# JialeTao/MRFA

Measured on AMD Instinct MI355X. Metric: frames/sec (256x256 source+driving pair) fwd+bwd, higher is better.
Workload: dtype f32; 1 GPU; vox1.yaml MTIA (TokenPose_B) prior + DenseMotion + RaftFlow refinement, 256x256, bs=8/GPU, fwd+bwd+clip+Adam, train-mode BN, surrogate L1 loss; global_batch=8, parallelism=dp1, prior=mtia, background_predictor=False, sync_bn=False, launch=hipGraph, optimizer=FlatAdam (K20), mfma=bf16x6

## Files before the change

### mrfa_amd/csrc/wgrad_lean.hip

```cpp
#include <stdlib.h>
#include <type_traits>
#include "mfma_bf16.h"

namespace {

constexpr int WL_MAXP = 24;

struct LeanW {
    const float* x; const float* dy; float* dw;
    const float* in_scale; const float* in_shift;
    int ldx, ldy, N, H, W, Cin, Cout, groups;
    float alpha;
    int G;
    int Q;
};
struct LeanWMulti {
    int n;
    int prefix[WL_MAXP + 1];
    LeanW p[WL_MAXP];
};

template <int NB, int TW, bool PRO, int NP>
__global__ __launch_bounds__(256, 1) void wgrad_lean_kernel(const LeanWMulti a) {
    constexpr int NPXW = NB == 1 ? 4 : 1;
    constexpr int TR = 32 / TW, PR = NPXW * TR, HP = TW + 2, HPIX = (PR + 2) * HP, DPIX = NPXW * 32;
    constexpr int XBLK = HPIX * 64, DBLK = DPIX * 64;
    constexpr int NPC = NP == 6 ? 3 : (NP == 3 ? 2 : 1);
    constexpr int XPLANE = NB * XBLK, DPLANE = NB * DBLK;
    constexpr int NXU = NB * HPIX * 8, NDU = NB * DPIX * 8;
    constexpr int NX = (NXU + 255) / 256, ND = (NDU + 255) / 256;
    extern __shared__ __attribute__((aligned(16))) unsigned char smem[];
    constexpr int IMG = NPC * (XPLANE + DPLANE);

    const int tid = threadIdx.x, lane = tid & 63, wave = __builtin_amdgcn_readfirstlane(tid >> 6);
    int pi = 0;
    while (pi + 1 < a.n && (int)blockIdx.x >= a.prefix[pi + 1]) ++pi;
    const LeanW& p = a.p[pi];
    const int local = (int)blockIdx.x - a.prefix[pi];
    const int nci = p.Cin / (32 * NB);
    const int bg = local / p.G, jr = local - bg * p.G;
    const int co0 = (bg / nci) * (32 * NB), ci0 = (bg % nci) * (32 * NB);
    const int q0 = (int)((long long)jr * p.Q / p.G), q1 = (int)((long long)(jr + 1) * p.Q / p.G);
    const int tiles_x = p.W / TW, tiles_y = (p.H + PR - 1) / PR;
    const int wpx = NB == 1 ? wave : 0, wco = NB == 1 ? 0 : (wave >> 1), wci = NB == 1 ? 0 : (wave & 1);

    auto x_unit = [&](int j, int& blk, int& hp, int& quad) -> bool {
        const int u = tid + j * 256;
        const int uu = u < NXU ? u : 0;
        blk = uu / (HPIX * 8);
        const int rem = uu - blk * (HPIX * 8);
        hp = rem >> 3;
        quad = rem & 7;
        return u < NXU;
    };
    auto d_unit = [&](int j, int& blk, int& px, int& quad) -> bool {
        const int u = tid + j * 256;
        const int uu = u < NDU ? u : 0;
        blk = uu / (DPIX * 8);
        const int rem = uu - blk * (DPIX * 8);
        px = rem >> 3;
        quad = rem & 7;
        return u < NDU;
    };
    float* const smP = reinterpret_cast<float*>(smem + 2 * IMG);
    if constexpr (PRO) {
        const int G = p.groups > 1 ? p.groups : 1;
        for (int i = tid; i < G * 2 * 32 * NB; i += 256) {
            const int g = i / (2 * 32 * NB), r = i - g * (2 * 32 * NB), which = r / (32 * NB), c = r - which * (32 * NB);
            smP[i] = (which ? p.in_shift : p.in_scale)[g * p.Cin + ci0 + c];
        }
        __syncthreads();
    }

    f32x4 rx[NX], rd[ND];
    unsigned okmask = 0;
    int cur_grp = 0;
    auto load_patch = [&](int q) {
        const int tx = q % tiles_x;
        int t = q / tiles_x;
        const int ty = t % tiles_y, n = t / tiles_y;
        const int y0 = ty * PR, x0 = tx * TW;
        const float* xb = p.x + (size_t)n * p.H * p.W * p.ldx;
        const float* db = p.dy + (size_t)n * p.H * p.W * p.ldy;
        okmask = 0;
#pragma unroll
        for (int j = 0; j < NX; ++j) {
            int blk, hp, quad;
            const bool val = x_unit(j, blk, hp, quad);
            const int hy = hp / HP, hx = hp - hy * HP;
            const int iy = y0 - 1 + hy, ix = x0 - 1 + hx;
            const bool ok = val && (unsigned)iy < (unsigned)p.H && (unsigned)ix < (unsigned)p.W;
            okmask |= ok ? (1u << j) : 0u;
            rx[j] = *reinterpret_cast<const f32x4*>(xb + (size_t)(ok ? iy * p.W + ix : 0) * p.ldx + ci0 + blk * 32 + quad * 4);
        }
#pragma unroll
        for (int j = 0; j < ND; ++j) {
            int blk, px, quad;
            const bool val = d_unit(j, blk, px, quad);
            const int r = px / TW, c = px - r * TW;
            const int oy = y0 + r;
            const bool ok = val && oy < p.H;
            okmask |= ok ? (1u << (16 + j)) : 0u;
            rd[j] = *reinterpret_cast<const f32x4*>(db + (size_t)(ok ? oy * p.W + x0 + c : 0) * p.ldy + co0 + blk * 32 + quad * 4);
        }
        cur_grp = p.groups > 1 ? n / (p.N / p.groups) : 0;
    };
    auto store_unit = [&](int k, int buf) {
        const f32x4 z = {0.f, 0.f, 0.f, 0.f};
        unsigned char* const smX = smem + buf * IMG;
        unsigned char* const smD = smX + NPC * XPLANE;
        if (k < NX) {
            const int j = k;
            int blk, hp, quad;
            const bool val = x_unit(j, blk, hp, quad);
            f32x4 v = rx[j];
            if constexpr (PRO) {
                const float* ps = smP + cur_grp * (2 * 32 * NB) + blk * 32 + quad * 4;
                const f32x4 psc = *reinterpret_cast<const f32x4*>(ps), psh = *reinterpret_cast<const f32x4*>(ps + 32 * NB);
                v = v * psc + psh;
#pragma unroll
                for (int e = 0; e < 4; ++e) v[e] = fmaxf(v[e], 0.f);
            }
            v = (okmask >> j) & 1u ? v : z;
            u32x2 p1, p2, p3;
            bf16_pieces<NP>(v, p1, p2, p3);
            if (val) {
                unsigned char* dst = smX + blk * XBLK + hp * 64 + quad * 8;
                *reinterpret_cast<u32x2*>(dst) = p1;
                if constexpr (NPC >= 2) *reinterpret_cast<u32x2*>(dst + XPLANE) = p2;
                if constexpr (NPC == 3) *reinterpret_cast<u32x2*>(dst + 2 * XPLANE) = p3;
            }
        } else {
            const int j = k - NX;
            int blk, px, quad;
            const bool val = d_unit(j, blk, px, quad);
            const f32x4 v = (okmask >> (16 + j)) & 1u ? rd[j] : z;
            u32x2 p1, p2, p3;
            bf16_pieces<NP>(v, p1, p2, p3);
            if (val) {
                unsigned char* dst = smD + blk * DBLK + px * 64 + quad * 8;
                *reinterpret_cast<u32x2*>(dst) = p1;
                if constexpr (NPC >= 2) *reinterpret_cast<u32x2*>(dst + DPLANE) = p2;
                if constexpr (NPC == 3) *reinterpret_cast<u32x2*>(dst + 2 * DPLANE) = p3;
            }
        }
    };

    f32x16 acc[9];
#pragma unroll
    for (int t = 0; t < 9; ++t)
#pragma unroll
        for (int r = 0; r < 16; ++r) acc[t][r] = 0.f;

    const int l16 = lane & 15, grp16 = lane >> 4;
    const int frag_off = (8 * (grp16 >> 1) + (l16 >> 2)) * 64 + (grp16 & 1) * 32 + (l16 & 3) * 8;
    const int a_off = wco * DBLK + wpx * (32 * 64) + frag_off;
    const int b_off = wci * XBLK + frag_off;
    constexpr int TG = 3, NGRP = 3;
    constexpr int NUNIT = NX + ND, UPG = (NUNIT + 2 * NGRP - 1) / (2 * NGRP);
    auto compute = [&](int buf, bool stage) {
        const unsigned char* const smX = smem + buf * IMG;
        const unsigned char* const smD = smX + NPC * XPLANE;
#pragma unroll
        for (int kk = 0; kk < 2; ++kk) {
            const int row0 = TW == 32 ? wpx : wpx * 2 + kk, col0 = TW == 32 ? 16 * kk : 0;
            bf16x8 af[NPC];
#pragma unroll
            for (int pc = 0; pc < NPC; ++pc) af[pc] = tr_frag(smD + pc * DPLANE + a_off + kk * 16 * 64);
#pragma unroll
            for (int gi = 0; gi < NGRP; ++gi) {
                const int g0 = gi * TG;
                bf16x8 bfr[NPC][TG];
#pragma unroll
                for (int q = 0; q < TG; ++q) {
                    const int tap = g0 + q, r = tap / 3, s = tap - 3 * r;
#pragma unroll
                    for (int pc = 0; pc < NPC; ++pc) bfr[pc][q] = tr_frag(smX + pc * XPLANE + b_off + ((row0 + r) * HP + col0 + s) * 64);
                }
#pragma unroll
                for (int t = 6 - NP; t < 6; ++t)
#pragma unroll
                    for (int q = 0; q < TG; ++q) acc[g0 + q] = __builtin_amdgcn_mfma_f32_32x32x16_bf16(af[PA[t]], bfr[PB[t]][q], acc[g0 + q], 0, 0, 0);
                if (stage) {
#pragma unroll
                    for (int k = (kk * NGRP + gi) * UPG; k < (kk * NGRP + gi + 1) * UPG; ++k)
                        if (k < NUNIT) store_unit(k, buf ^ 1);
                }
            }
        }
    };

    if (q0 < q1) {
        load_patch(q0);
#pragma unroll
        for (int k = 0; k < NUNIT; ++k) store_unit(k, q0 & 1);
        if (q0 + 1 < q1) load_patch(q0 + 1);
        __syncthreads();
        for (int q = q0; q < q1; ++q) {
            const bool more = q + 1 < q1;
            compute(q & 1, more);
            if (q + 2 < q1) load_patch(q + 2);
            __syncthreads();
        }
    }

    if constexpr (NB == 1) {
        float* red = reinterpret_cast<float*>(smem);
        for (int w = 1; w < 4; ++w) {
            __syncthreads();
            if (wave == w) {
#pragma unroll
                for (int t = 0; t < 9; ++t)
#pragma unroll
                    for (int r = 0; r < 16; ++r) red[(t * 16 + r) * 64 + lane] = acc[t][r];
            }
            __syncthreads();
            if (wave == 0) {
#pragma unroll
                for (int t = 0; t < 9; ++t)
#pragma unroll
                    for (int r = 0; r < 16; ++r) acc[t][r] += red[(t * 16 + r) * 64 + lane];
            }
        }
        if (wave != 0) return;
    }
    if (q0 >= q1) return;
    const int ci = ci0 + wci * 32 + (lane & 31), half = lane >> 5;
#pragma unroll
    for (int t = 0; t < 9; ++t)
#pragma unroll
        for (int g = 0; g < 4; ++g)
#pragma unroll
            for (int e = 0; e < 4; ++e) {
                const int co = co0 + wco * 32 + 8 * g + 4 * half + e;
                atomicAdd(p.dw + ((size_t)t * p.Cout + co) * p.Cin + ci, p.alpha * acc[t][4 * g + e]);
            }
}

template <int NB, int TW>
constexpr size_t wl_lds(int npc) {
    constexpr int NPXW = NB == 1 ? 4 : 1, TR = 32 / TW, PR = NPXW * TR, HP = TW + 2, HPIX = (PR + 2) * HP, DPIX = NPXW * 32;
    const size_t st = (size_t)2 * npc * NB * (HPIX + DPIX) * 64 + (size_t)3 * 2 * 32 * NB * 4, red = NB == 1 ? (size_t)9 * 16 * 64 * 4 : 0;
    return st > red ? st : red;
}

int wl_variant(const mrfa_wgrad_params& p) {
    if (p.Cin == 32 && p.Cout == 32) return (p.Wout % 32) == 0 ? 0 : -1;
    if ((p.Cin % 64) || (p.Cout % 64)) return -1;
    return (p.Wout % 32) == 0 ? 1 : ((p.Wout % 16) == 0 ? 2 : -1);
}

template <int NB, int TW>
int wl_launch(hipStream_t st, const LeanWMulti& m, bool pro, int mode) {
    dim3 grid((unsigned)m.prefix[m.n]);
#define WL(PRO_, NP_)                                                                                                                              \
    do {                                                                                                                                          \
        constexpr size_t lds = wl_lds<NB, TW>(NP_ == 6 ? 3 : (NP_ == 3 ? 2 : 1));                                                                  \
        if constexpr (lds > 65536) {                                        \
            static const hipError_t attr = hipFuncSetAttribute(reinterpret_cast<const void*>(&wgrad_lean_kernel<NB, TW, PRO_, NP_>),               \
                                                               hipFuncAttributeMaxDynamicSharedMemorySize, (int)lds);                             \
            if (attr != hipSuccess) { mrfa_set_error("wgrad(lean): %zu bytes of LDS refused: %s", lds, hipGetErrorString(attr)); return 2; }      \
        }                                                                                                                                         \
        hipLaunchKernelGGL((wgrad_lean_kernel<NB, TW, PRO_, NP_>), grid, dim3(256), lds, st, m);                                                  \
    } while (0)
    if (mode == 3) { if (pro) WL(true, 1); else WL(false, 1); }
    else if (mode == 2) { if (pro) WL(true, 3); else WL(false, 3); }
    else { if (pro) WL(true, 6); else WL(false, 6); }
#undef WL
    return 0;
}

}

bool mrfa_wgrad_lean_eligible(const mrfa_wgrad_params& p) {
    const int mode = mrfa_get_mfma_mode();
    if (!g_tune.wgrad_lean || (mode != 1 && mode != 2 && mode != 3)) return false;
    if (p.kflat > 0 || p.ups || p.R != 3 || p.S != 3 || p.pad != 1 || p.nbatch > 1 || p.ksplit > 0 || p.stride > 1 || p.dbias) return false;
    if (p.Hout != p.Hin || p.Wout != p.Win || p.Cin > 128 || p.Cout > 128) return false;
    if ((p.ldx % 4) != 0 || !aligned16(p.x) || (p.ldy % 4) != 0 || !aligned16(p.dy)) return false;
    if (p.in_scale && (!p.in_relu || !aligned16(p.in_scale) || !aligned16(p.in_shift))) return false;
    if (p.groups > 1 && ((p.N % p.groups) != 0 || p.groups > 3)) return false;
    if ((long long)p.N * p.Hin * p.Win * p.ldx >= (1ll << 31) || (long long)p.N * p.Hout * p.Wout * p.ldy >= (1ll << 31)) return false;
    if (2.0 * (double)p.N * p.Hout * p.Wout * p.Cout * 9.0 * p.Cin > 2.6e9) return false;
    return wl_variant(p) >= 0;
}

int mrfa_wgrad_lean_multi(hipStream_t st, const mrfa_wgrad_params* ps, int n, unsigned char* taken) {
    const int mode = mrfa_get_mfma_mode();
    int neligible = 0;
    for (int i = 0; i < n; ++i) neligible += (taken[i] = mrfa_wgrad_lean_eligible(ps[i]) ? 1 : 0);
    if (!neligible) return 0;
    for (int v = 0; v < 3; ++v)
        for (int pro = 0; pro < 2; ++pro) {
            int idx[4096], cnt = 0;
            for (int i = 0; i < n && cnt < 4096; ++i)
                if (taken[i] && wl_variant(ps[i]) == v && (ps[i].in_scale != nullptr) == (pro != 0)) idx[cnt++] = i;
            for (int b0 = 0; b0 < cnt; b0 += WL_MAXP) {
                const int nb = cnt - b0 < WL_MAXP ? cnt - b0 : WL_MAXP;
                LeanWMulti m;
                m.n = nb;
                m.prefix[0] = 0;
                long long blocks = 0;
                for (int k = 0; k < nb; ++k) {
                    const mrfa_wgrad_params& q = ps[idx[b0 + k]];
                    blocks += v == 0 ? 1 : (q.Cin / 64) * (q.Cout / 64);
                }
                int G = (int)((512 + blocks - 1) / blocks);
                if (G > 64) G = 64;
                for (int k = 0; k < nb; ++k) {
                    const mrfa_wgrad_params& q = ps[idx[b0 + k]];
                    LeanW& w = m.p[k];
                    const int PR = v == 0 ? 4 : (v == 1 ? 1 : 2), TW = v == 2 ? 16 : 32;
                    w.x = q.x; w.dy = q.dy; w.dw = q.dw; w.in_scale = q.in_scale; w.in_shift = q.in_shift;
                    w.ldx = q.ldx; w.ldy = q.ldy; w.N = q.N; w.H = q.Hout; w.W = q.Wout; w.Cin = q.Cin; w.Cout = q.Cout; w.groups = q.groups;
                    w.alpha = q.alpha;
                    w.Q = q.N * (q.Wout / TW) * cdiv(q.Hout, PR);
                    w.G = G < w.Q ? G : w.Q;
                    const int nblocks = v == 0 ? 1 : (q.Cin / 64) * (q.Cout / 64);
                    m.prefix[k + 1] = m.prefix[k] + w.G * nblocks;
                }
                int rc = 0;
                if (v == 0) rc = wl_launch<1, 32>(st, m, pro != 0, mode);
                else if (v == 1) rc = wl_launch<2, 32>(st, m, pro != 0, mode);
                else rc = wl_launch<2, 16>(st, m, pro != 0, mode);
                if (rc) return rc;
                MRFA_CHECK_LAUNCH("mrfa_conv2d_wgrad_multi(lean)");
            }
        }
    return 0;
}
```

Before: 103.1 pairs/s.

## Split wgrad taps across two wave groups in 512-thread lean kernel

Doubles the lean weight-gradient workgroup to 512 threads. The 9 filter taps are split between two groups of four waves, one taking 5 taps and the other 4, which cuts per-wave accumulator registers from 9 to 5 tiles. For the NB=2 variants the pixel patch per iteration is doubled (two k-tiles), and the grid target is lowered to 256 workgroups so each block covers more patches. This aims to lift register pressure and improve latency hiding, at the cost of duplicated A-fragment loads across the tap groups, larger LDS tiles and fewer blocks in flight.

```diff
diff --git a/mrfa_amd/csrc/wgrad_lean.hip b/mrfa_amd/csrc/wgrad_lean.hip
--- a/mrfa_amd/csrc/wgrad_lean.hip
+++ b/mrfa_amd/csrc/wgrad_lean.hip
@@ -20,15 +20,20 @@
     LeanW p[WL_MAXP];
 };
 
+constexpr int WL_TARGET_WGS = 256;
+constexpr int WL_THREADS = 512;
+constexpr int WL_TAPS = 5;
+
 template <int NB, int TW, bool PRO, int NP>
-__global__ __launch_bounds__(256, 1) void wgrad_lean_kernel(const LeanWMulti a) {
+__global__ __launch_bounds__(WL_THREADS, 1) void wgrad_lean_kernel(const LeanWMulti a) {
     constexpr int NPXW = NB == 1 ? 4 : 1;
-    constexpr int TR = 32 / TW, PR = NPXW * TR, HP = TW + 2, HPIX = (PR + 2) * HP, DPIX = NPXW * 32;
+    constexpr int NKT = NB == 1 ? 1 : 2;
+    constexpr int TR = 32 / TW, PR = NPXW * NKT * TR, HP = TW + 2, HPIX = (PR + 2) * HP, DPIX = NPXW * NKT * 32;
     constexpr int XBLK = HPIX * 64, DBLK = DPIX * 64;
     constexpr int NPC = NP == 6 ? 3 : (NP == 3 ? 2 : 1);
     constexpr int XPLANE = NB * XBLK, DPLANE = NB * DBLK;
     constexpr int NXU = NB * HPIX * 8, NDU = NB * DPIX * 8;
-    constexpr int NX = (NXU + 255) / 256, ND = (NDU + 255) / 256;
+    constexpr int NX = (NXU + WL_THREADS - 1) / WL_THREADS, ND = (NDU + WL_THREADS - 1) / WL_THREADS;
     extern __shared__ __attribute__((aligned(16))) unsigned char smem[];
     constexpr int IMG = NPC * (XPLANE + DPLANE);
 
@@ -42,10 +47,13 @@
     const int co0 = (bg / nci) * (32 * NB), ci0 = (bg % nci) * (32 * NB);
     const int q0 = (int)((long long)jr * p.Q / p.G), q1 = (int)((long long)(jr + 1) * p.Q / p.G);
     const int tiles_x = p.W / TW, tiles_y = (p.H + PR - 1) / PR;
-    const int wpx = NB == 1 ? wave : 0, wco = NB == 1 ? 0 : (wave >> 1), wci = NB == 1 ? 0 : (wave & 1);
+    const int tg = wave >> 2, w4 = wave & 3;
+    const int wpx = NB == 1 ? w4 : 0, wco = NB == 1 ? 0 : (w4 >> 1), wci = NB == 1 ? 0 : (w4 & 1);
+    const int t0 = tg * WL_TAPS;
+    const bool five = tg == 0;
 
     auto x_unit = [&](int j, int& blk, int& hp, int& quad) -> bool {
-        const int u = tid + j * 256;
+        const int u = tid + j * WL_THREADS;
         const int uu = u < NXU ? u : 0;
         blk = uu / (HPIX * 8);
         const int rem = uu - blk * (HPIX * 8);
@@ -54,7 +62,7 @@
         return u < NXU;
     };
     auto d_unit = [&](int j, int& blk, int& px, int& quad) -> bool {
-        const int u = tid + j * 256;
+        const int u = tid + j * WL_THREADS;
         const int uu = u < NDU ? u : 0;
         blk = uu / (DPIX * 8);
         const int rem = uu - blk * (DPIX * 8);
@@ -65,7 +73,7 @@
     float* const smP = reinterpret_cast<float*>(smem + 2 * IMG);
     if constexpr (PRO) {
         const int G = p.groups > 1 ? p.groups : 1;
-        for (int i = tid; i < G * 2 * 32 * NB; i += 256) {
+        for (int i = tid; i < G * 2 * 32 * NB; i += WL_THREADS) {
             const int g = i / (2 * 32 * NB), r = i - g * (2 * 32 * NB), which = r / (32 * NB), c = r - which * (32 * NB);
             smP[i] = (which ? p.in_shift : p.in_scale)[g * p.Cin + ci0 + c];
         }
@@ -146,41 +154,49 @@
         }
     };
 
-    f32x16 acc[9];
-#pragma unroll
-    for (int t = 0; t < 9; ++t)
+    f32x16 acc[WL_TAPS];
+#pragma unroll
+    for (int t = 0; t < WL_TAPS; ++t)
 #pragma unroll
         for (int r = 0; r < 16; ++r) acc[t][r] = 0.f;
 
     const int l16 = lane & 15, grp16 = lane >> 4;
     const int frag_off = (8 * (grp16 >> 1) + (l16 >> 2)) * 64 + (grp16 & 1) * 32 + (l16 & 3) * 8;
     const int a_off = wco * DBLK + wpx * (32 * 64) + frag_off;
-    const int b_off = wci * XBLK + frag_off;
-    constexpr int TG = 3, NGRP = 3;
-    constexpr int NUNIT = NX + ND, UPG = (NUNIT + 2 * NGRP - 1) / (2 * NGRP);
+    int b_off[WL_TAPS];
+#pragma unroll
+    for (int j = 0; j < WL_TAPS; ++j) {
+        const int ta = j, tb = WL_TAPS + (j < 4 ? j : 3);
+        const int toff = five ? ((ta / 3) * HP + ta % 3) * 64 : ((tb / 3) * HP + tb % 3) * 64;
+        b_off[j] = wci * XBLK + wpx * (TR * HP * 64) + frag_off + toff;
+    }
+    constexpr int NGRP = 2;
+    constexpr int NKK = 2 * NKT;
+    constexpr int NUNIT = NX + ND, UPG = (NUNIT + NKK * NGRP - 1) / (NKK * NGRP);
     auto compute = [&](int buf, bool stage) {
         const unsigned char* const smX = smem + buf * IMG;
         const unsigned char* const smD = smX + NPC * XPLANE;
 #pragma unroll
-        for (int kk = 0; kk < 2; ++kk) {
-            const int row0 = TW == 32 ? wpx : wpx * 2 + kk, col0 = TW == 32 ? 16 * kk : 0;
+        for (int kk = 0; kk < NKK; ++kk) {
+            const int xstep = ((16 * kk / TW) * HP + 16 * kk % TW) * 64;
             bf16x8 af[NPC];
 #pragma unroll
             for (int pc = 0; pc < NPC; ++pc) af[pc] = tr_frag(smD + pc * DPLANE + a_off + kk * 16 * 64);
 #pragma unroll
             for (int gi = 0; gi < NGRP; ++gi) {
-                const int g0 = gi * TG;
+                constexpr int TG = 3;
+                const int g0 = gi * TG, gn = gi == 0 ? TG : WL_TAPS - TG;
                 bf16x8 bfr[NPC][TG];
 #pragma unroll
-                for (int q = 0; q < TG; ++q) {
-                    const int tap = g0 + q, r = tap / 3, s = tap - 3 * r;
-#pragma unroll
-                    for (int pc = 0; pc < NPC; ++pc) bfr[pc][q] = tr_frag(smX + pc * XPLANE + b_off + ((row0 + r) * HP + col0 + s) * 64);
-                }
+                for (int q = 0; q < gn; ++q)
+#pragma unroll
+                    for (int pc = 0; pc < NPC; ++pc) bfr[pc][q] = tr_frag(smX + pc * XPLANE + b_off[g0 + q] + xstep);
 #pragma unroll
                 for (int t = 6 - NP; t < 6; ++t)
 #pragma unroll
-                    for (int q = 0; q < TG; ++q) acc[g0 + q] = __builtin_amdgcn_mfma_f32_32x32x16_bf16(af[PA[t]], bfr[PB[t]][q], acc[g0 + q], 0, 0, 0);
+                    for (int q = 0; q < gn; ++q)
+                        if (g0 + q < WL_TAPS - 1 || five)
+                            acc[g0 + q] = __builtin_amdgcn_mfma_f32_32x32x16_bf16(af[PA[t]], bfr[PB[t]][q], acc[g0 + q], 0, 0, 0);
                 if (stage) {
 #pragma unroll
                     for (int k = (kk * NGRP + gi) * UPG; k < (kk * NGRP + gi + 1) * UPG; ++k)
@@ -205,42 +221,44 @@
     }
 
     if constexpr (NB == 1) {
-        float* red = reinterpret_cast<float*>(smem);
+        float* red = reinterpret_cast<float*>(smem) + tg * (WL_TAPS * 16 * 64);
         for (int w = 1; w < 4; ++w) {
             __syncthreads();
-            if (wave == w) {
-#pragma unroll
-                for (int t = 0; t < 9; ++t)
+            if (wpx == w) {
+#pragma unroll
+                for (int t = 0; t < WL_TAPS; ++t)
 #pragma unroll
                     for (int r = 0; r < 16; ++r) red[(t * 16 + r) * 64 + lane] = acc[t][r];
             }
             __syncthreads();
-            if (wave == 0) {
-#pragma unroll
-                for (int t = 0; t < 9; ++t)
+            if (wpx == 0) {
+#pragma unroll
+                for (int t = 0; t < WL_TAPS; ++t)
 #pragma unroll
                     for (int r = 0; r < 16; ++r) acc[t][r] += red[(t * 16 + r) * 64 + lane];
             }
         }
-        if (wave != 0) return;
+        if (wpx != 0) return;
     }
     if (q0 >= q1) return;
     const int ci = ci0 + wci * 32 + (lane & 31), half = lane >> 5;
 #pragma unroll
-    for (int t = 0; t < 9; ++t)
+    for (int t = 0; t < WL_TAPS; ++t) {
+        if (t == WL_TAPS - 1 && !five) break;
 #pragma unroll
         for (int g = 0; g < 4; ++g)
 #pragma unroll
             for (int e = 0; e < 4; ++e) {
                 const int co = co0 + wco * 32 + 8 * g + 4 * half + e;
-                atomicAdd(p.dw + ((size_t)t * p.Cout + co) * p.Cin + ci, p.alpha * acc[t][4 * g + e]);
-            }
+                atomicAdd(p.dw + ((size_t)(t0 + t) * p.Cout + co) * p.Cin + ci, p.alpha * acc[t][4 * g + e]);
+            }
+    }
 }
 
 template <int NB, int TW>
 constexpr size_t wl_lds(int npc) {
-    constexpr int NPXW = NB == 1 ? 4 : 1, TR = 32 / TW, PR = NPXW * TR, HP = TW + 2, HPIX = (PR + 2) * HP, DPIX = NPXW * 32;
-    const size_t st = (size_t)2 * npc * NB * (HPIX + DPIX) * 64 + (size_t)3 * 2 * 32 * NB * 4, red = NB == 1 ? (size_t)9 * 16 * 64 * 4 : 0;
+    constexpr int NPXW = NB == 1 ? 4 : 1, NKT = NB == 1 ? 1 : 2, TR = 32 / TW, PR = NPXW * NKT * TR, HP = TW + 2, HPIX = (PR + 2) * HP, DPIX = NPXW * NKT * 32;
+    const size_t st = (size_t)2 * npc * NB * (HPIX + DPIX) * 64 + (size_t)3 * 2 * 32 * NB * 4, red = NB == 1 ? (size_t)2 * WL_TAPS * 16 * 64 * 4 : 0;
     return st > red ? st : red;
 }
 
@@ -261,7 +279,7 @@
                                                                hipFuncAttributeMaxDynamicSharedMemorySize, (int)lds);                             \
             if (attr != hipSuccess) { mrfa_set_error("wgrad(lean): %zu bytes of LDS refused: %s", lds, hipGetErrorString(attr)); return 2; }      \
         }                                                                                                                                         \
-        hipLaunchKernelGGL((wgrad_lean_kernel<NB, TW, PRO_, NP_>), grid, dim3(256), lds, st, m);                                                  \
+        hipLaunchKernelGGL((wgrad_lean_kernel<NB, TW, PRO_, NP_>), grid, dim3(WL_THREADS), lds, st, m);                                                  \
     } while (0)
     if (mode == 3) { if (pro) WL(true, 1); else WL(false, 1); }
     else if (mode == 2) { if (pro) WL(true, 3); else WL(false, 3); }
@@ -305,12 +323,13 @@
                     const mrfa_wgrad_params& q = ps[idx[b0 + k]];
                     blocks += v == 0 ? 1 : (q.Cin / 64) * (q.Cout / 64);
                 }
-                int G = (int)((512 + blocks - 1) / blocks);
+                int G = (int)(WL_TARGET_WGS / blocks);
+                if (G < 1) G = 1;
                 if (G > 64) G = 64;
                 for (int k = 0; k < nb; ++k) {
                     const mrfa_wgrad_params& q = ps[idx[b0 + k]];
                     LeanW& w = m.p[k];
-                    const int PR = v == 0 ? 4 : (v == 1 ? 1 : 2), TW = v == 2 ? 16 : 32;
+                    const int PR = v == 0 ? 4 : (v == 1 ? 2 : 4), TW = v == 2 ? 16 : 32;
                     w.x = q.x; w.dy = q.dy; w.dw = q.dw; w.in_scale = q.in_scale; w.in_shift = q.in_shift;
                     w.ldx = q.ldx; w.ldy = q.ldy; w.N = q.N; w.H = q.Hout; w.W = q.Wout; w.Cin = q.Cin; w.Cout = q.Cout; w.groups = q.groups;
                     w.alpha = q.alpha;
```

Result: no change. 102.7 pairs/s (-0.4%).
